# Arthur151/ROMP

Hardware: NVIDIA H100
Metric: frames/sec 512x512 ROMP-HRNet32 (whole hot path) (higher is better)
Workload: dtype bf16

## Files before the change

romp_b200/_lib.py:

```python
from __future__ import annotations

import ctypes as C
import os
import subprocess
import sys

HERE = os.path.dirname(os.path.abspath(__file__))
ROOT = os.path.dirname(HERE)
LIB_PATH = os.path.join(HERE, "lib", "libb200romp.so")
CSRC = os.path.join(HERE, "csrc")
SOURCES = ["net.cu", "conv_simt.cu", "conv_tc.cu", "conv_block_tc.cu", "conv_stem_tc.cu", "conv1d_tc.cu", "parse.cu", "smpl.cu", "smpl_blend_tc.cu", "project.cu", "bev.cu", "pack.cu", "preproc.cu", "temporal.cu", "resnet_ops.cu"]

F32, BF16, U8 = 0, 1, 2
ENGINE_AUTO, ENGINE_SIMT, ENGINE_WGMMA, ENGINE_TF32 = 0, 1, 2, 3
ENGINE_TCGEN05 = ENGINE_WGMMA


class ConvDesc(C.Structure):
    _fields_ = [(n, C.c_int) for n in (
        "in_", "in_c_off", "out", "out_c_off", "res", "res_c_off", "res_broadcast", "cin", "cout",
        "ksize", "stride", "relu", "upsample", "input_norm", "pow_channel", "engine")]


class SumDesc(C.Structure):
    _fields_ = [("out", C.c_int), ("base", C.c_int), ("n_terms", C.c_int), ("term", C.c_int * 4), ("up", C.c_int * 4),
                ("relu", C.c_int), ("term_c_off", C.c_int * 4)]


class BevWeights(C.Structure):
    _fields_ = [(n, C.POINTER(C.c_float)) for n in (
        "center_ref", "cam_ref", "coordmap", "anchors", "embed", "w0", "b0", "w1", "b1", "w2", "b2")]


NVCC_FLAGS = ["-Xcompiler", "-fPIC", "-std=c++17", "-O3", "-lineinfo", "-gencode", "arch=compute_90a,code=sm_90a"]
OBJ_DIR = os.path.join(HERE, "lib", "obj")


def _nvcc():
    return os.environ.get("NVCC", "/usr/local/cuda/bin/nvcc")


def nvcc_command(out_path=LIB_PATH):
    return [_nvcc(), "-shared"] + NVCC_FLAGS + ["-o", out_path] + [os.path.join(CSRC, s) for s in SOURCES]

# ... 143 lines not shown
```

romp_b200/csrc/conv_tc.cu:

```cuda
#include <mutex>

#include "conv_tc.cuh"
#include "tc_device.cuh"

namespace b200romp {

thread_local int g_tc_pdl_override = -1;

constexpr int kTcThreads = 384;
constexpr int kMaxRings = 2;

__host__ __device__ constexpr int s2_row_bytes(int cin, int eb) { return cin * eb >= 512 ? 64 : (cin * eb < 128 ? cin * eb : 128); }

__host__ __device__ constexpr int tc_num_rings(int stages) { return stages >= 4 ? kMaxRings : 1; }
__host__ __device__ constexpr int tc_ring_size(int stages, int ring) { return tc_num_rings(stages) == 1 ? stages : (stages + 1 - ring) / 2; }
__host__ __device__ constexpr int tc_ring_base(int stages, int ring) { return ring ? (stages + 1) / 2 : 0; }

template <int MODE, int CIN, int NT, int EB>
struct TcCfg {
  static constexpr bool S2 = MODE == 2;
  static constexpr int KS = MODE == 1 ? 1 : 3;
  static constexpr int TAPS = KS * KS;
  static constexpr int PAD = KS / 2;
  static constexpr int ROWB = S2 ? s2_row_bytes(CIN, EB) : tc_row_bytes(KS, CIN, EB);
// ... 263 lines not shown
  return true;
}

bool tc_conv_supported(const ConvParams& p, int ksize, int stride) {
  TcConvPlan plan;
  return tc_shape_supported(p, ksize, stride) && tc_tile(p, ksize, stride, &plan);
}

template <int MODE, int CIN, int NT, int EB>
static int launch_inst(const TcConvPlan& plan, const ConvParams& p, cudaStream_t stream, bool set_attr_only) {
  if (set_attr_only) {
    B2R_CUDA_OK(cudaFuncSetAttribute(conv_tc_kernel<MODE, CIN, NT, EB, true>, cudaFuncAttributeMaxDynamicSharedMemorySize, 227 * 1024));
    B2R_CUDA_OK(cudaFuncSetAttribute(conv_tc_kernel<MODE, CIN, NT, EB, false>, cudaFuncAttributeMaxDynamicSharedMemorySize, 227 * 1024));
    return B200ROMP_OK;
  }
  auto kern = p.cout % NT == 0 && tc_nhwc_out(p, p.cout) ? conv_tc_kernel<MODE, CIN, NT, EB, false> : conv_tc_kernel<MODE, CIN, NT, EB, true>;
  CUtensorMap tm;
  memcpy(&tm, plan.tmap_in, sizeof(tm));
  S2Maps s2;
  memcpy(&s2, plan.tmap_s2, sizeof(s2));
  const int tiles_x = p.Wout / 8, tiles_y = p.Hout / 16;
  const int num_tiles = tiles_x * tiles_y * p.B;
  dim3 grid(std::min(plan.grid_x, num_tiles), plan.grid_y);
  B2R_CUDA_OK(tc_launch(kern, grid, kTcThreads, plan.smem_bytes, stream, tm, s2, p, reinterpret_cast<const uint8_t*>(plan.d_wpack), tiles_x,
                        tiles_y, num_tiles, plan.stages, plan.kmask));
  return B200ROMP_OK;
}

static int dispatch(const TcConvPlan& plan, const ConvParams& p, cudaStream_t stream, bool attr) {
  const int mode = plan.kind == 32 ? 2 : plan.kind / 10;
#define B2R_CASE(M, C, N, E) \
  if (mode == M && plan.cin == C && plan.nt == N && plan.eb == E) return launch_inst<M, C, N, E>(plan, p, stream, attr);
  B2R_CASE(3, 32, 32, 2) B2R_CASE(3, 32, 64, 2) B2R_CASE(3, 64, 32, 2) B2R_CASE(3, 64, 64, 2) B2R_CASE(3, 128, 32, 2) B2R_CASE(3, 128, 64, 2)
  B2R_CASE(3, 256, 32, 2) B2R_CASE(3, 256, 64, 2)
  B2R_CASE(1, 32, 32, 2) B2R_CASE(1, 32, 64, 2) B2R_CASE(1, 64, 32, 2) B2R_CASE(1, 64, 64, 2) B2R_CASE(1, 128, 32, 2) B2R_CASE(1, 128, 64, 2)
  B2R_CASE(1, 256, 32, 2) B2R_CASE(1, 256, 64, 2)
  B2R_CASE(2, 32, 32, 2) B2R_CASE(2, 32, 64, 2) B2R_CASE(2, 64, 32, 2) B2R_CASE(2, 64, 64, 2) B2R_CASE(2, 128, 32, 2) B2R_CASE(2, 256, 32, 2)
  B2R_CASE(3, 32, 32, 4) B2R_CASE(3, 32, 64, 4) B2R_CASE(3, 64, 32, 4) B2R_CASE(3, 64, 64, 4) B2R_CASE(3, 128, 32, 4) B2R_CASE(3, 256, 16, 4)
  B2R_CASE(1, 32, 32, 4) B2R_CASE(1, 32, 64, 4) B2R_CASE(1, 64, 32, 4) B2R_CASE(1, 64, 64, 4) B2R_CASE(1, 128, 32, 4) B2R_CASE(1, 128, 64, 4)
  B2R_CASE(1, 256, 32, 4) B2R_CASE(1, 256, 64, 4)
  B2R_CASE(2, 32, 32, 4) B2R_CASE(2, 32, 64, 4) B2R_CASE(2, 64, 32, 4) B2R_CASE(2, 128, 32, 4)
#undef B2R_CASE
  set_error("conv_tc: no instantiation for mode %d cin%d nt%d eb%d", mode, plan.cin, plan.nt, plan.eb);
  return B200ROMP_EINVAL;
}

int tc_conv_prepare(const ConvParams& p, int ksize, int stride, const float* w_oihw, int sm_count, TcConvPlan* plan,
                    std::vector<void*>* allocs) {
  PFN_encodeTiled encode = tc_get_encode();
  if (!encode) {
    set_error("conv_tc: cuTensorMapEncodeTiled is unavailable");
    return B200ROMP_ECUDA;
  }
  if (!tc_tile(p, ksize, stride, plan)) {
    set_error("conv_tc: k%d s%d cin%d does not fit shared memory", ksize, stride, p.cin);
    return B200ROMP_EINVAL;
  }
  const int eb = plan->eb, rowb = tc_rowb(ksize, stride, p.cin, eb), cw = rowb / eb;
  plan->grid_y = (p.cout + plan->nt - 1) / plan->nt;
  plan->grid_x = std::max(1, sm_count / plan->grid_y);
  int rc = tc_pack_weights(w_oihw, p.cin, p.cout, ksize * ksize, plan->nt, &plan->d_wpack, allocs, rowb, eb);
  if (rc) return rc;
  const CUtensorMapDataType dtype = eb == 2 ? CU_TENSOR_MAP_DATA_TYPE_BFLOAT16 : CU_TENSOR_MAP_DATA_TYPE_FLOAT32;
  const CUtensorMapSwizzle swizzle = rowb == 128 ? CU_TENSOR_MAP_SWIZZLE_128B : CU_TENSOR_MAP_SWIZZLE_64B;
  if (stride == 2) {
    const cuuint64_t C = (cuuint64_t)p.in_C;
    const cuuint64_t gdim[5] = {2 * C, (cuuint64_t)p.Win / 2, 2, (cuuint64_t)p.Hin / 2, (cuuint64_t)p.B};
    const cuuint64_t E = (cuuint64_t)eb;
    const cuuint64_t gstr[4] = {2 * C * E, (cuuint64_t)p.Win * C * E, 2 * (cuuint64_t)p.Win * C * E, (cuuint64_t)p.Hin * p.Win * C * E};
    const cuuint32_t estr[5] = {1, 1, 1, 1, 1};
    for (int i = 0; i < 4; ++i) {
      const cuuint32_t box[5] = {(cuuint32_t)cw, (cuuint32_t)((i & 1) ? 8 : 9), 1, (cuuint32_t)(i < 2 ? 17 : 16), 1};
      CUtensorMap tm;
      CUresult cr = encode(&tm, dtype, 5, const_cast<void*>(p.in), gdim, gstr, box, estr, CU_TENSOR_MAP_INTERLEAVE_NONE, swizzle,
                           CU_TENSOR_MAP_L2_PROMOTION_L2_128B, CU_TENSOR_MAP_FLOAT_OOB_FILL_NONE);
      if (cr != CUDA_SUCCESS) {
        set_error("conv_tc: cuTensorMapEncodeTiled (stride 2) failed with %d", (int)cr);
        return B200ROMP_ECUDA;
      }
      memcpy(plan->tmap_s2[i], &tm, sizeof(tm));
    }
  } else {
    const int hh = 16 + 2 * (ksize / 2), hw = 8 + 2 * (ksize / 2);
    CUtensorMap tm;
    const cuuint64_t gdim[4] = {(cuuint64_t)p.cin, (cuuint64_t)p.Win, (cuuint64_t)p.Hin, (cuuint64_t)p.B};
    const cuuint64_t gstr[3] = {(cuuint64_t)p.in_C * eb, (cuuint64_t)p.Win * p.in_C * eb, (cuuint64_t)p.Hin * p.Win * p.in_C * eb};
    const cuuint32_t box[4] = {(cuuint32_t)cw, (cuuint32_t)hw, (cuuint32_t)hh, 1};
    const cuuint32_t estr[4] = {1, 1, 1, 1};
    void* base = const_cast<uint8_t*>(static_cast<const uint8_t*>(p.in) + (size_t)p.in_c_off * eb);
    CUresult cr = encode(&tm, dtype, 4, base, gdim, gstr, box, estr, CU_TENSOR_MAP_INTERLEAVE_NONE, swizzle,
                         CU_TENSOR_MAP_L2_PROMOTION_L2_128B, CU_TENSOR_MAP_FLOAT_OOB_FILL_NONE);
    if (cr != CUDA_SUCCESS) {
      set_error("conv_tc: cuTensorMapEncodeTiled failed with %d", (int)cr);
      return B200ROMP_ECUDA;
    }
    memcpy(plan->tmap_in, &tm, sizeof(tm));
  }
  return dispatch(*plan, p, nullptr, true);
}

int tc_conv_launch(const TcConvPlan& plan, const ConvParams& p, cudaStream_t stream) { return dispatch(plan, p, stream, false); }

}
```

romp_b200/csrc/conv_tc.cuh:

```cuda
#pragma once
#include <cuda.h>

#include <string>
#include <vector>

#include "common.cuh"

namespace b200romp {

struct S2Maps {
  CUtensorMap m[4];
};

struct TcConvPlan {
  int kind = 0;
  int cin = 0, cout = 0, nt = 0;
  int eb = 2;
  int grid_x = 0, grid_y = 0, stages = 0;
  int smem_bytes = 0;
  void* d_wpack = nullptr;
  alignas(64) unsigned char tmap_in[128];
  alignas(64) unsigned char tmap_s2[4][128];
  unsigned kmask = 0xFFFFFFFFu;
  const void* encoded_in = nullptr;
  int encoded_batch = 0;
  void* d_wpack2 = nullptr;
  const float* d_bias1 = nullptr;
  int fold = 0;
  std::string describe() const;
};

bool tc_conv_supported(const ConvParams& p, int ksize, int stride);
int tc_conv_prepare(const ConvParams& p, int ksize, int stride, const float* w_oihw, int sm_count, TcConvPlan* plan,
                    std::vector<void*>* allocs);
int tc_conv_launch(const TcConvPlan& plan, const ConvParams& p, cudaStream_t stream);
bool tc_conv1d_supported(const ConvParams& p);
int tc_conv1d_prepare(const ConvParams& p, const float* w_oi3, int sm_count, TcConvPlan* plan, std::vector<void*>* allocs);
int tc_conv1d_launch(TcConvPlan& plan, const ConvParams& p, cudaStream_t stream);
bool tc_stem_supported(const ConvParams& p, int ksize, int stride);
int tc_stem_prepare(const ConvParams& p, const float* w_oihw, int sm_count, TcConvPlan* plan, std::vector<void*>* allocs);
int tc_stem_launch(const TcConvPlan& plan, const ConvParams& p, cudaStream_t stream);
bool tc_block_supported(const ConvParams& p);
int tc_block_prepare(const ConvParams& p, const float* w1_oihw, const float* b1, const float* w2_oihw, int sm_count,
                     TcConvPlan* plan, std::vector<void*>* allocs);
int tc_block_launch(const TcConvPlan& plan, const ConvParams& p, cudaStream_t stream);

}
```

romp_b200/csrc/net.cu:

```cuda
#include <stdarg.h>
#include <stdlib.h>
#include <string.h>

#include <algorithm>
#include <map>
#include <mutex>
#include <vector>

#include "common.cuh"
#include "conv_tc.cuh"

namespace b200romp {

static thread_local std::string g_last_error;

void set_error(const char* fmt, ...) {
  char buf[1024];
  va_list ap;
  va_start(ap, fmt);
  vsnprintf(buf, sizeof(buf), fmt, ap);
  va_end(ap);
  g_last_error = buf;
}

struct Tensor {
  int H, W, C, dtype, nchw, external;
  void* ptr = nullptr;
  bool constant = false;
  int first_def = -1, last_use = -1;
  size_t frame_bytes() const { return (size_t)H * W * C * dtype_size(dtype); }
};

enum class Kernel { Sum, MaxPool, Simt, Generic7x7, Deconv4x4, Wgmma, WgmmaStem, WgmmaConv1d, WgmmaBlock };

struct Op {
  Kernel kernel = Kernel::Simt;
  b200romp_sum_desc sum;
  b200romp_conv_desc d;
  std::vector<float> w_host, b_host;
  float* d_w_simt = nullptr;
  float* d_bias = nullptr;
  int coutPad = 0;
  TcConvPlan tc;
  int lane = 0;
  int mid = -1;
  std::vector<float> w2_host, b2_host;
};

static bool on_wgmma(Kernel k) { return k == Kernel::Wgmma || k == Kernel::WgmmaStem || k == Kernel::WgmmaConv1d || k == Kernel::WgmmaBlock; }

}

using namespace b200romp;

struct b200romp_net {
  int device = 0;
  int sm_count = 132;
  bool finalized = false;
  int max_batch = 0;
  std::vector<Tensor> tensors;
  std::vector<Op> ops;
  std::vector<void*> device_allocs;
  char* workspace = nullptr;
  size_t workspace_bytes = 0;
  struct GraphKey {
    int batch;
    std::vector<void*> ext;
    bool operator<(const GraphKey& o) const { return batch != o.batch ? batch < o.batch : ext < o.ext; }
  };
  std::map<GraphKey, cudaGraphExec_t> graphs;
  bool use_graph = true;
  static constexpr int kLanes = 4;
  cudaStream_t lane_stream[kLanes] = {nullptr, nullptr, nullptr, nullptr};
  std::vector<cudaEvent_t> op_done;
  cudaEvent_t fork_ev = nullptr;
  bool use_lanes = false;
};

static int fill_params(const b200romp_net* net, const Op& op, int batch, bool allow_unbound, ConvParams* out) {
  const b200romp_conv_desc& d = op.d;
  const Tensor& ti = net->tensors[d.in];
  const Tensor& to = net->tensors[d.out];
// ... 190 lines not shown
  for (int k = 0; k < p.n_terms; ++k) {
    const Tensor& tt = net->tensors[op.sum.term[k]];
    B2R_REQUIRE(tt.ptr, "sum op: unbound term tensor");
    p.term[k] = tt.ptr; p.term_dt[k] = tt.dtype; p.up[k] = op.sum.up[k];
    p.term_C[k] = tt.C; p.term_c_off[k] = op.sum.term_c_off[k];
  }
  p.B = batch; p.H = to.H; p.W = to.W; p.C = to.C; p.relu = op.sum.relu;
  *out = p;
  return B200ROMP_OK;
}

static int enqueue_op(b200romp_net* net, Op& op, int batch, cudaStream_t stream) {
  ConvParams p;
  if (op.kernel != Kernel::Sum && op.kernel != Kernel::MaxPool) {
    int rc = fill_params(net, op, batch, false, &p);
    if (rc) return rc;
  }
  switch (op.kernel) {
    case Kernel::Sum: {
      SumParams sp;
      int rc = fill_sum_params(net, op, batch, &sp);
      return rc ? rc : launch_fuse_sum(sp, stream);
    }
    case Kernel::MaxPool: {
      const Tensor& ti = net->tensors[op.d.in];
      const Tensor& to = net->tensors[op.d.out];
      B2R_REQUIRE(ti.ptr && to.ptr, "maxpool op: unbound tensor");
      return launch_maxpool3x3s2(ti.ptr, to.ptr, ti.dtype, batch, ti.H, ti.W, ti.C, stream);
    }
    case Kernel::Simt: return launch_conv_simt(p, op.d.ksize, op.d.stride, stream);
    case Kernel::Generic7x7: return launch_conv_generic(p, 7, op.d.stride, stream);
    case Kernel::Deconv4x4: return launch_deconv4x4s2(p, stream);
    case Kernel::Wgmma: return tc_conv_launch(op.tc, p, stream);
    case Kernel::WgmmaStem: return tc_stem_launch(op.tc, p, stream);
    case Kernel::WgmmaConv1d: return tc_conv1d_launch(op.tc, p, stream);
    case Kernel::WgmmaBlock: return tc_block_launch(op.tc, p, stream);
  }
  return B200ROMP_EINVAL;
}

static int upload(b200romp_net* net, const std::vector<float>& v, float** d) {
  B2R_CUDA_OK(cudaMalloc(d, v.size() * sizeof(float)));
  net->device_allocs.push_back(*d);
  B2R_CUDA_OK(cudaMemcpy(*d, v.data(), v.size() * sizeof(float), cudaMemcpyHostToDevice));
  return B200ROMP_OK;
}

static bool fold_eligible(const b200romp_net* net, const Op& op) {
  static const bool off = [] { const char* e = getenv("B200ROMP_TC_NO_FOLD"); return e && e[0] == '1'; }();
  const b200romp_conv_desc& d = op.d;
  const Tensor& ti = net->tensors[d.in];
  const Tensor& to = net->tensors[d.out];
  if (off || d.ksize != 3 || d.stride != 1 || d.upsample != 1 || d.cin != 32 || d.cout != 32) return false;
  if (ti.C != 32 || to.C != 32 || d.in_c_off || d.out_c_off || ti.external || to.external) return false;
  if (ti.dtype != B200ROMP_BF16 || to.dtype != B200ROMP_BF16 || to.nchw || d.pow_channel >= 0 || d.input_norm) return false;
  if (ti.W % 16 != 0 || ti.H % 16 != 0) return false;
  if (d.res >= 0) {
    const Tensor& tr = net->tensors[d.res];
    if (tr.C != 32 || d.res_c_off || d.res_broadcast || tr.dtype != B200ROMP_BF16 || tr.external) return false;
  }
  return true;
}

static void fold_pixel_pairs(std::vector<float>* w, std::vector<float>* b) {
  std::vector<float> w2((size_t)64 * 64 * 9, 0.f), b2(64);
  for (int dx = 0; dx < 2; ++dx)
// ... 73 lines not shown
          f.w2_host = std::move(b.w_host);
          f.b2_host = std::move(b.b_host);
          fused.push_back(std::move(f));
          ++i;
          continue;
        }
      }
    }
    fused.push_back(std::move(a));
  }
  net->ops = std::move(fused);
}

static int choose_kernel(const b200romp_net* net, int i, Op& op) {
  const b200romp_conv_desc& d = op.d;
  const Tensor& ti = net->tensors[d.in];
  const Tensor& to = net->tensors[d.out];
  if (d.ksize == 7 || d.ksize == 42) {
    op.kernel = d.ksize == 7 ? Kernel::Generic7x7 : Kernel::Deconv4x4;
    return B200ROMP_OK;
  }
  op.kernel = Kernel::Simt;
  const bool forced = d.engine == B200ROMP_ENGINE_WGMMA;
  const bool stem = ti.dtype == B200ROMP_U8 && d.cin == 3 && d.ksize == 3 && d.stride == 2;
  if (!forced && !(d.engine == B200ROMP_ENGINE_TF32 && ti.dtype == B200ROMP_F32) &&
      !(d.engine == B200ROMP_ENGINE_AUTO && (ti.dtype == B200ROMP_BF16 || stem)))
    return B200ROMP_OK;
  ConvParams p;
  fill_params(net, op, net->max_batch, true, &p);
  if (stem) {
    if (!to.external && d.res < 0 && tc_stem_supported(p, d.ksize, d.stride)) op.kernel = Kernel::WgmmaStem;
  } else if (d.ksize == 13) {
    if (tc_conv1d_supported(p)) op.kernel = Kernel::WgmmaConv1d;
  } else if (!ti.external && tc_conv_supported(p, d.ksize, d.stride)) {
    op.kernel = Kernel::Wgmma;
    op.tc.fold = fold_eligible(net, op);
  }
  if (forced && op.kernel == Kernel::Simt) {
    set_error("op %d: tensor-core engine forced but shape unsupported", i);
    return B200ROMP_EINVAL;
  }
  return B200ROMP_OK;
}

static int prepare_op(b200romp_net* net, Op& op) {
  if (op.kernel == Kernel::Sum || op.kernel == Kernel::MaxPool) return B200ROMP_OK;
  const b200romp_conv_desc& d = op.d;
  std::vector<float> w = std::move(op.w_host), b = std::move(op.b_host), w2 = std::move(op.w2_host), b2 = std::move(op.b2_host);
  if (op.tc.fold) {
    fold_pixel_pairs(&w, &b);
    if (op.kernel == Kernel::WgmmaBlock) fold_pixel_pairs(&w2, &b2);
  }
  std::vector<float> bias = op.kernel == Kernel::WgmmaBlock ? b2 : b;
  op.coutPad = ((int)bias.size() + 63) / 64 * 64;
  bias.resize(op.coutPad, 0.f);
  int rc = upload(net, bias, &op.d_bias);
  if (rc) return rc;
  ConvParams p;
  fill_params(net, op, net->max_batch, true, &p);
  switch (op.kernel) {
    case Kernel::Simt:
    case Kernel::Generic7x7:
    case Kernel::Deconv4x4: {
      const int taps = conv_taps(d.ksize);
      std::vector<float> packed((size_t)taps * d.cin * op.coutPad, 0.f);
      for (int co = 0; co < d.cout; ++co)
        for (int ci = 0; ci < d.cin; ++ci)
          for (int t = 0; t < taps; ++t)
            packed[((size_t)t * d.cin + ci) * op.coutPad + co] =
                d.ksize == 42 ? w[((size_t)ci * d.cout + co) * taps + t] : w[((size_t)co * d.cin + ci) * taps + t];
      return upload(net, packed, &op.d_w_simt);
    }
    case Kernel::Wgmma:
      if (op.tc.fold) op.tc.kmask = fold_kmask();
      return tc_conv_prepare(p, d.ksize, d.stride, w.data(), net->sm_count, &op.tc, &net->device_allocs);
    case Kernel::WgmmaStem: return tc_stem_prepare(p, w.data(), net->sm_count, &op.tc, &net->device_allocs);
    case Kernel::WgmmaConv1d: return tc_conv1d_prepare(p, w.data(), net->sm_count, &op.tc, &net->device_allocs);
    case Kernel::WgmmaBlock: return tc_block_prepare(p, w.data(), b.data(), w2.data(), net->sm_count, &op.tc, &net->device_allocs);
    default: return B200ROMP_OK;
  }
}

int b200romp_net_finalize(b200romp_net* net, int max_batch) {
  B2R_REQUIRE(net && !net->finalized && max_batch > 0, "finalize: bad arguments");
  B2R_CUDA_OK(cudaSetDevice(net->device));
  fuse_basic_blocks(net);
  const int nT = (int)net->tensors.size(), nO = (int)net->ops.size();
  for (int i = 0; i < nO; ++i) {
    const b200romp_conv_desc& d = net->ops[i].d;
    Tensor& to = net->tensors[d.out];
    if (to.first_def < 0) to.first_def = i;
    to.last_use = std::max(to.last_use, i);
    net->tensors[d.in].last_use = std::max(net->tensors[d.in].last_use, i);
    if (d.res >= 0) net->tensors[d.res].last_use = std::max(net->tensors[d.res].last_use, i);
    if (net->ops[i].kernel == Kernel::Sum)
      for (int k = 0; k < net->ops[i].sum.n_terms; ++k) {
        Tensor& tt = net->tensors[net->ops[i].sum.term[k]];
        B2R_REQUIRE(tt.external || tt.constant || (tt.first_def >= 0 && tt.first_def < i), "op %d sums tensor %d before it is written", i, net->ops[i].sum.term[k]);
        tt.last_use = std::max(tt.last_use, i);
      }
  }
  for (int i = 0; i < nO; ++i) {
    const b200romp_conv_desc& d = net->ops[i].d;
    const Tensor& ti = net->tensors[d.in];
    B2R_REQUIRE(ti.external || ti.constant || (ti.first_def >= 0 && ti.first_def < i), "op %d reads tensor %d before it is written", i, d.in);
    if (d.res >= 0) {
      const Tensor& tr = net->tensors[d.res];
      B2R_REQUIRE(tr.external || tr.constant || (tr.first_def >= 0 && tr.first_def < i), "op %d adds tensor %d before it is written", i, d.res);
// ... 305 lines not shown
```

romp_b200/csrc/tc_device.cuh:

```cuda
#pragma once
#include <cuda.h>

#include <vector>

#include "conv_tc.cuh"

namespace b200romp {

__device__ __forceinline__ uint32_t smem_u32(const void* p) { return (uint32_t)__cvta_generic_to_shared(p); }

__device__ __forceinline__ void mbar_init(uint64_t* bar, uint32_t count) {
  asm volatile("mbarrier.init.shared::cta.b64 [%0], %1;" ::"r"(smem_u32(bar)), "r"(count) : "memory");
}
__device__ __forceinline__ void mbar_arrive_expect_tx(uint64_t* bar, uint32_t bytes) {
  asm volatile("mbarrier.arrive.expect_tx.shared::cta.b64 _, [%0], %1;" ::"r"(smem_u32(bar)), "r"(bytes) : "memory");
}
__device__ __forceinline__ void mbar_arrive(uint64_t* bar) {
  asm volatile("mbarrier.arrive.shared::cta.b64 _, [%0];" ::"r"(smem_u32(bar)) : "memory");
}
__device__ __forceinline__ bool mbar_try_wait(uint64_t* bar, uint32_t parity) {
  uint32_t ok;
  asm volatile(
      "{\n\t.reg .pred p;\n\t"
      "mbarrier.try_wait.parity.shared::cta.b64 p, [%1], %2;\n\t"
// ... 20 lines not shown
__device__ __forceinline__ void fence_barrier_init() { asm volatile("fence.mbarrier_init.release.cluster;" ::: "memory"); }
__device__ __forceinline__ void fence_proxy_async() { asm volatile("fence.proxy.async.shared::cta;" ::: "memory"); }
__device__ __forceinline__ void wg_bar_sync(int id) { asm volatile("bar.sync %0, 128;" ::"r"(id) : "memory"); }

__device__ __forceinline__ uint64_t l2_policy_stream() {
  uint64_t pol;
  asm volatile("createpolicy.fractional.L2::evict_normal.b64 %0, 1.0;" : "=l"(pol));
  return pol;
}
__device__ __forceinline__ void tma_load_3d(void* dst, const CUtensorMap* map, uint64_t* bar, int c0, int c1, int c2, uint64_t pol) {
  asm volatile(
      "cp.async.bulk.tensor.3d.shared::cluster.global.mbarrier::complete_tx::bytes.L2::cache_hint [%0], [%1, {%3, %4, %5}], [%2], %6;"
      ::"r"(smem_u32(dst)), "l"(map), "r"(smem_u32(bar)), "r"(c0), "r"(c1), "r"(c2), "l"(pol)
      : "memory");
}
__device__ __forceinline__ void tma_load_4d(void* dst, const CUtensorMap* map, uint64_t* bar, int c0, int c1, int c2, int c3, uint64_t pol) {
  asm volatile(
      "cp.async.bulk.tensor.4d.shared::cluster.global.mbarrier::complete_tx::bytes.L2::cache_hint [%0], [%1, {%3, %4, %5, %6}], [%2], %7;"
      ::"r"(smem_u32(dst)), "l"(map), "r"(smem_u32(bar)), "r"(c0), "r"(c1), "r"(c2), "r"(c3), "l"(pol)
      : "memory");
}
__device__ __forceinline__ void tma_load_5d(void* dst, const CUtensorMap* map, uint64_t* bar, int c0, int c1, int c2, int c3,
                                            int c4, uint64_t pol) {
  asm volatile(
      "cp.async.bulk.tensor.5d.shared::cluster.global.mbarrier::complete_tx::bytes.L2::cache_hint [%0], [%1, {%3, %4, %5, %6, %7}], [%2], %8;"
      ::"r"(smem_u32(dst)), "l"(map), "r"(smem_u32(bar)), "r"(c0), "r"(c1), "r"(c2), "r"(c3), "r"(c4), "l"(pol)
      : "memory");
}
__device__ __forceinline__ void bulk_copy_g2s(void* dst, const void* src, uint32_t bytes, uint64_t* bar) {
  asm volatile("cp.async.bulk.shared::cluster.global.mbarrier::complete_tx::bytes [%0], [%1], %2, [%3];"
               ::"r"(smem_u32(dst)), "l"(src), "r"(bytes), "r"(smem_u32(bar))
               : "memory");
}

__device__ __forceinline__ void wgmma_fence() { asm volatile("wgmma.fence.sync.aligned;" ::: "memory"); }
__device__ __forceinline__ void wgmma_commit() { asm volatile("wgmma.commit_group.sync.aligned;" ::: "memory"); }
template <int N>
__device__ __forceinline__ void wgmma_wait() { asm volatile("wgmma.wait_group.sync.aligned %0;" ::"n"(N) : "memory"); }

#define B2R_WG_R8(i) "+f"(d[i + 0]), "+f"(d[i + 1]), "+f"(d[i + 2]), "+f"(d[i + 3]), "+f"(d[i + 4]), "+f"(d[i + 5]), "+f"(d[i + 6]), "+f"(d[i + 7])
__device__ __forceinline__ void wgmma_n16(float (&d)[8], uint64_t a, uint64_t b, uint32_t scale_d, bool tf32) {
  if (!tf32)
    asm volatile(
        "{\n\t.reg .pred p;\n\tsetp.ne.b32 p, %10, 0;\n\t"
        "wgmma.mma_async.sync.aligned.m64n16k16.f32.bf16.bf16 {%0, %1, %2, %3, %4, %5, %6, %7}, %8, %9, p, 1, 1, 0, 0;\n\t}"
        : B2R_WG_R8(0)
        : "l"(a), "l"(b), "r"(scale_d)
        : "memory");
  else
    asm volatile(
        "{\n\t.reg .pred p;\n\tsetp.ne.b32 p, %10, 0;\n\t"
        "wgmma.mma_async.sync.aligned.m64n16k8.f32.tf32.tf32 {%0, %1, %2, %3, %4, %5, %6, %7}, %8, %9, p, 1, 1;\n\t}"
        : B2R_WG_R8(0)
        : "l"(a), "l"(b), "r"(scale_d)
        : "memory");
}
__device__ __forceinline__ void wgmma_n32(float (&d)[16], uint64_t a, uint64_t b, uint32_t scale_d, bool tf32) {
  if (!tf32)
    asm volatile(
        "{\n\t.reg .pred p;\n\tsetp.ne.b32 p, %18, 0;\n\t"
        "wgmma.mma_async.sync.aligned.m64n32k16.f32.bf16.bf16 {%0, %1, %2, %3, %4, %5, %6, %7, %8, %9, %10, %11, %12, %13, %14, %15}, "
        "%16, %17, p, 1, 1, 0, 0;\n\t}"
        : B2R_WG_R8(0), B2R_WG_R8(8)
        : "l"(a), "l"(b), "r"(scale_d)
        : "memory");
  else
    asm volatile(
        "{\n\t.reg .pred p;\n\tsetp.ne.b32 p, %18, 0;\n\t"
        "wgmma.mma_async.sync.aligned.m64n32k8.f32.tf32.tf32 {%0, %1, %2, %3, %4, %5, %6, %7, %8, %9, %10, %11, %12, %13, %14, %15}, "
        "%16, %17, p, 1, 1;\n\t}"
        : B2R_WG_R8(0), B2R_WG_R8(8)
        : "l"(a), "l"(b), "r"(scale_d)
        : "memory");
}
__device__ __forceinline__ void wgmma_n64(float (&d)[32], uint64_t a, uint64_t b, uint32_t scale_d, bool tf32) {
  if (!tf32)
    asm volatile(
        "{\n\t.reg .pred p;\n\tsetp.ne.b32 p, %34, 0;\n\t"
        "wgmma.mma_async.sync.aligned.m64n64k16.f32.bf16.bf16 {%0, %1, %2, %3, %4, %5, %6, %7, %8, %9, %10, %11, %12, %13, %14, "
        "%15, %16, %17, %18, %19, %20, %21, %22, %23, %24, %25, %26, %27, %28, %29, %30, %31}, %32, %33, p, 1, 1, 0, 0;\n\t}"
        : B2R_WG_R8(0), B2R_WG_R8(8), B2R_WG_R8(16), B2R_WG_R8(24)
        : "l"(a), "l"(b), "r"(scale_d)
        : "memory");
  else
    asm volatile(
        "{\n\t.reg .pred p;\n\tsetp.ne.b32 p, %34, 0;\n\t"
        "wgmma.mma_async.sync.aligned.m64n64k8.f32.tf32.tf32 {%0, %1, %2, %3, %4, %5, %6, %7, %8, %9, %10, %11, %12, %13, %14, "
        "%15, %16, %17, %18, %19, %20, %21, %22, %23, %24, %25, %26, %27, %28, %29, %30, %31}, %32, %33, p, 1, 1;\n\t}"
        : B2R_WG_R8(0), B2R_WG_R8(8), B2R_WG_R8(16), B2R_WG_R8(24)
        : "l"(a), "l"(b), "r"(scale_d)
        : "memory");
}
#undef B2R_WG_R8
template <int NT, int EB>
__device__ __forceinline__ void wgmma_any(float (&d)[NT / 2], uint64_t a, uint64_t b, uint32_t scale_d) {
  if constexpr (NT == 64) wgmma_n64(d, a, b, scale_d, EB == 4);
  else if constexpr (NT == 32) wgmma_n32(d, a, b, scale_d, EB == 4);
  else wgmma_n16(d, a, b, scale_d, EB == 4);
}

constexpr uint32_t kSw128 = 1, kSw64 = 2;
__device__ __forceinline__ uint64_t make_smem_desc(uint32_t addr, uint32_t sbo_bytes, uint32_t layout) {
  return (uint64_t)((addr & 0x3FFFF) >> 4) | ((uint64_t)1 << 16) | ((uint64_t)(sbo_bytes >> 4) << 32) | ((uint64_t)layout << 62);
}
__host__ __device__ constexpr uint32_t tc_layout(int row_bytes) { return row_bytes == 128 ? kSw128 : kSw64; }

__host__ __device__ constexpr int tc_row_bytes(int ksize, int cin, int eb) {
  return (ksize == 3 && cin >= 128) ? 64 : (cin * eb < 128 ? cin * eb : 128);
}

__device__ __forceinline__ uint32_t tf32_rna(uint32_t x) {
  uint32_t y;
  asm("cvt.rna.tf32.f32 %0, %1;" : "=r"(y) : "r"(x));
  return y;
}
__device__ __forceinline__ void tf32_round_smem(uint8_t* base, int bytes, int t, int nthreads) {
  const uint32_t s0 = smem_u32(base);
  for (int off = t * 16; off < bytes; off += nthreads * 16) {
    uint32_t a, b, c, d;
    asm volatile("ld.shared.v4.b32 {%0, %1, %2, %3}, [%4];" : "=r"(a), "=r"(b), "=r"(c), "=r"(d) : "r"(s0 + off));
    a = tf32_rna(a); b = tf32_rna(b); c = tf32_rna(c); d = tf32_rna(d);
    asm volatile("st.shared.v4.b32 [%4], {%0, %1, %2, %3};" ::"r"(a), "r"(b), "r"(c), "r"(d), "r"(s0 + off) : "memory");
  }
}
// ... 115 lines not shown
        const float b0 = __ldg(bias + c), b1 = __ldg(bias + c + 1);
#pragma unroll
        for (int e = 0; e < 2; ++e) {
          const int m = 64 * h + 16 * w + (l >> 2) + 8 * e;
          wg_store2(p, n, linear ? y0 : y0 + (m >> 3), linear ? x0 + m : x0 + (m & 7), c, acc[h][4 * j + 2 * e] + b0,
                    acc[h][4 * j + 2 * e + 1] + b1);
        }
      }
    }
  }
}

template <typename... KArgs, typename... Args>
static inline cudaError_t tc_launch(void (*kern)(KArgs...), dim3 grid, int threads, int smem_bytes, cudaStream_t stream, Args&&... args) {
  static const bool pdl_default = [] { const char* e = getenv("B200ROMP_NO_PDL"); return !(e && e[0] == '1'); }();
  const bool pdl = pdl_default && g_tc_pdl_override != 0;
  cudaLaunchConfig_t cfg = {};
  cfg.gridDim = grid;
  cfg.blockDim = dim3(threads);
  cfg.dynamicSmemBytes = (size_t)smem_bytes;
  cfg.stream = stream;
  cudaLaunchAttribute at[1];
  at[0].id = cudaLaunchAttributeProgrammaticStreamSerialization;
  at[0].val.programmaticStreamSerializationAllowed = 1;
  cfg.attrs = at;
  cfg.numAttrs = pdl ? 1 : 0;
  return cudaLaunchKernelEx(&cfg, kern, static_cast<KArgs>(args)...);
}

typedef CUresult (*PFN_encodeTiled)(CUtensorMap*, CUtensorMapDataType, cuuint32_t, void*, const cuuint64_t*, const cuuint64_t*,
                                    const cuuint32_t*, const cuuint32_t*, CUtensorMapInterleave, CUtensorMapSwizzle,
                                    CUtensorMapL2promotion, CUtensorMapFloatOOBfill);
PFN_encodeTiled tc_get_encode();
int tc_pack_weights(const float* w_oihw, int cin, int cout, int taps, int nt, void** d_out, std::vector<void*>* allocs, int rowb, int eb);
float tc_round_tf32_host(float w);

}
```

Baseline: 2687.

## Add warp-specialized N=128 WGMMA kernel for deep 3x3 convs sharing weight stages

Adds a dedicated 3x3 stride-1 bf16 conv kernel for cin 128/256 with cout a multiple of 128. It uses two consumer warpgroups, each working on its own 16x8 output tile, which share a deep ring of streamed weight stages, plus per-consumer halo TMA producers and setmaxnreg register rebalancing. The wider n128 tile and shared weight fetch are meant to cut weight traffic and raise tensor-core utilisation on the low-resolution HRNet branches. The risks are lower occupancy from a single large-smem block per SM, the lag handshake between consumers stalling them, and removal of the old cin256/nt64 instantiation.

Measured after the change: 2727, median of 6. +1.5%, better.

```diff
diff --git a/romp_b200/_lib.py b/romp_b200/_lib.py
--- a/romp_b200/_lib.py
+++ b/romp_b200/_lib.py
@@ -9,7 +9,7 @@
 ROOT = os.path.dirname(HERE)
 LIB_PATH = os.path.join(HERE, "lib", "libb200romp.so")
 CSRC = os.path.join(HERE, "csrc")
-SOURCES = ["net.cu", "conv_simt.cu", "conv_tc.cu", "conv_block_tc.cu", "conv_stem_tc.cu", "conv1d_tc.cu", "parse.cu", "smpl.cu", "smpl_blend_tc.cu", "project.cu", "bev.cu", "pack.cu", "preproc.cu", "temporal.cu", "resnet_ops.cu"]
+SOURCES = ["net.cu", "conv_simt.cu", "conv_tc.cu", "conv_deep_tc.cu", "conv_block_tc.cu", "conv_stem_tc.cu", "conv1d_tc.cu", "parse.cu", "smpl.cu", "smpl_blend_tc.cu", "project.cu", "bev.cu", "pack.cu", "preproc.cu", "temporal.cu", "resnet_ops.cu"]
 
 F32, BF16, U8 = 0, 1, 2
 ENGINE_AUTO, ENGINE_SIMT, ENGINE_WGMMA, ENGINE_TF32 = 0, 1, 2, 3
diff --git a/romp_b200/csrc/conv_deep_tc.cu b/romp_b200/csrc/conv_deep_tc.cu
--- /dev/null
+++ b/romp_b200/csrc/conv_deep_tc.cu
@@ -0,0 +1,207 @@
+#include "conv_tc.cuh"
+#include "tc_device.cuh"
+
+namespace b200romp {
+
+namespace {
+constexpr int kThreads = 384;
+constexpr int kNT = 128;
+constexpr int kRowB = 64;
+constexpr int kCW = kRowB / 2;
+constexpr int kHaloPayload = 18 * 10 * kRowB;
+constexpr int kHaloBytes = 12 * 1024;
+constexpr int kWBytes = kNT * kRowB;
+constexpr int kConsumers = 2;
+constexpr int kHaloStages = 2;
+constexpr int kBarBytes = 1024;
+constexpr int kWStages = (227 * 1024 - 1024 - kBarBytes - kConsumers * kHaloStages * kHaloBytes) / kWBytes;
+constexpr int kLag = 18;
+constexpr int kSmemBytes = 1024  + kConsumers * kHaloStages * kHaloBytes + kWStages * kWBytes + kBarBytes;
+static_assert(kSmemBytes <= 227 * 1024, "deep conv stages exceed shared memory");
+static_assert((2 * kConsumers * kHaloStages + 2 * kWStages + 1) * 8 <= kBarBytes, "barriers exceed their block");
+static_assert(kLag < kWStages, "the lag must leave consumer 0 a free weight stage");
+}
+
+template <int CIN>
+__global__ void __launch_bounds__(kThreads, 1)
+conv_deep_tc_kernel(const __grid_constant__ CUtensorMap tmap, const ConvParams p, const uint8_t* __restrict__ wpack, int tiles_x,
+                    int tiles_y, int num_tiles) {
+  constexpr int KCH = CIN / kCW;
+  static_assert(kLag < 9 * KCH, "consumer 0 must reach the lag inside its first tile");
+  extern __shared__ uint8_t smem_raw[];
+  uint8_t* smem = reinterpret_cast<uint8_t*>((reinterpret_cast<uintptr_t>(smem_raw) + 1023) & ~(uintptr_t)1023);
+  uint8_t* sH = smem;
+  uint8_t* sW = sH + kConsumers * kHaloStages * kHaloBytes;
+  uint64_t* hfull = reinterpret_cast<uint64_t*>(sW + kWStages * kWBytes);
+  uint64_t* hempty = hfull + kConsumers * kHaloStages;
+  uint64_t* wfull = hempty + kConsumers * kHaloStages;
+  uint64_t* wempty = wfull + kWStages;
+  uint64_t* go = wempty + kWStages;
+
+  const int warp = threadIdx.x >> 5;
+  if (threadIdx.x == 0) {
+    for (int i = 0; i < kConsumers * kHaloStages; ++i) {
+      mbar_init(&hfull[i], 1);
+      mbar_init(&hempty[i], 4);
+    }
+    for (int i = 0; i < kWStages; ++i) {
+      mbar_init(&wfull[i], 1);
+      mbar_init(&wempty[i], 4 * kConsumers);
+    }
+    mbar_init(go, 4);
+    fence_barrier_init();
+  }
+  __syncthreads();
+  pdl_trigger();
+  const int per_frame = tiles_x * tiles_y;
+  const int n_pairs = (num_tiles + 1) / 2;
+
+  if (warp < 4) {
+    setmaxnreg_dec<40>();
+    if (warp < kConsumers) {
+      const int g = warp;
+      const bool leader = (threadIdx.x & 31) == 0;
+      pdl_wait();
+      const uint64_t pol = l2_policy_stream();
+      int hs = 0;
+      uint32_t hph = 0;
+      for (int pair = blockIdx.x; pair < n_pairs; pair += gridDim.x) {
+        const int tile = min(2 * pair + g, num_tiles - 1);
+        const int n = tile / per_frame, rem = tile % per_frame;
+        for (int c = 0; c < KCH; ++c) {
+          const int hidx = g * kHaloStages + hs;
+          mbar_wait(&hempty[hidx], hph ^ 1);
+          if (leader) {
+            mbar_arrive_expect_tx(&hfull[hidx], kHaloPayload);
+            tma_load_4d(sH + (size_t)hidx * kHaloBytes, &tmap, &hfull[hidx], c * kCW, (rem % tiles_x) * 8 - 1, (rem / tiles_x) * 16 - 1,
+                        n, pol);
+          }
+          __syncwarp();
+          if (++hs == kHaloStages) { hs = 0; hph ^= 1; }
+        }
+      }
+    } else if (warp == kConsumers) {
+      const bool leader = (threadIdx.x & 31) == 0;
+      const uint8_t* wsrc = wpack + (size_t)blockIdx.y * 9 * KCH * kWBytes;
+      int ws = 0;
+      uint32_t wph = 0;
+      for (int pair = blockIdx.x; pair < n_pairs; pair += gridDim.x) {
+        for (int c = 0; c < KCH; ++c) {
+          for (int tap = 0; tap < 9; ++tap) {
+            mbar_wait(&wempty[ws], wph ^ 1);
+            if (leader) {
+              mbar_arrive_expect_tx(&wfull[ws], kWBytes);
+              bulk_copy_g2s(sW + (size_t)ws * kWBytes, wsrc + (size_t)(tap * KCH + c) * kWBytes, kWBytes, &wfull[ws]);
+            }
+            __syncwarp();
+            if (++ws == kWStages) { ws = 0; wph ^= 1; }
+          }
+        }
+      }
+    }
+  } else {
+    setmaxnreg_inc<232>();
+    const int g = (warp >> 2) - 1, t = threadIdx.x & 127, wlane = threadIdx.x & 31;
+    pdl_wait();
+    if (g == 1) mbar_wait(go, 0);
+    const uint32_t h_base = smem_u32(sH + (size_t)g * kHaloStages * kHaloBytes), w_base = smem_u32(sW);
+    int hs = 0, ws = 0, done = 0;
+    uint32_t hph = 0, wph = 0;
+    for (int pair = blockIdx.x; pair < n_pairs; pair += gridDim.x) {
+      const int tile = 2 * pair + g;
+      const int tc = min(tile, num_tiles - 1);
+      const int n = tc / per_frame, rem = tc % per_frame;
+      const int y0 = (rem / tiles_x) * 16, x0 = (rem % tiles_x) * 8;
+      float acc[2][kNT / 2];
+#pragma unroll
+      for (int h = 0; h < 2; ++h)
+#pragma unroll
+        for (int j = 0; j < kNT / 2; ++j) acc[h][j] = 0.f;
+      uint32_t scale_d = 0;
+      int prev_w = -1, prev_h = -1;
+      for (int c = 0; c < KCH; ++c) {
+        const int hidx = g * kHaloStages + hs;
+        mbar_wait(&hfull[hidx], hph);
+        const uint32_t a_base = h_base + (uint32_t)(hs * kHaloBytes);
+#pragma unroll
+        for (int tap = 0; tap < 9; ++tap) {
+          mbar_wait(&wfull[ws], wph);
+          const uint32_t a_tap = a_base + (uint32_t)(((tap / 3) * 10 + tap % 3) * kRowB), sbo = 10 * kRowB;
+          const uint32_t b_tap = w_base + (uint32_t)(ws * kWBytes);
+          wgmma_fence();
+#pragma unroll
+          for (int k = 0; k < kRowB / 32; ++k) {
+            const uint64_t bdesc = make_smem_desc(b_tap + k * 32, 8 * kRowB, kSw64);
+            wgmma_n128(acc[0], make_smem_desc(a_tap + k * 32, sbo, kSw64), bdesc, scale_d);
+            wgmma_n128(acc[1], make_smem_desc(a_tap + 8 * sbo + k * 32, sbo, kSw64), bdesc, scale_d);
+            scale_d = 1;
+          }
+          wgmma_commit();
+          if (prev_w >= 0) {
+            wgmma_wait<1>();
+            if (wlane == 0) {
+              mbar_arrive(&wempty[prev_w]);
+              if (prev_h >= 0) mbar_arrive(&hempty[prev_h]);
+            }
+          }
+          prev_w = ws;
+          prev_h = tap == 8 ? hidx : -1;
+          if (++ws == kWStages) { ws = 0; wph ^= 1; }
+          if (g == 0 && ++done == kLag && wlane == 0) mbar_arrive(go);
+        }
+        if (++hs == kHaloStages) { hs = 0; hph ^= 1; }
+      }
+      wgmma_wait<0>();
+      if (wlane == 0) {
+        mbar_arrive(&wempty[prev_w]);
+        mbar_arrive(&hempty[prev_h]);
+      }
+      if (tile < num_tiles) wg_epilogue<kNT, kEpiNhwc>(p, acc, p.bias, n, y0, x0, blockIdx.y * kNT, t);
+    }
+  }
+}
+
+bool tc_deep_supported(const ConvParams& p, int ksize, int stride, int sm_count) {
+  if (ksize != 3 || stride != 1 || p.in_dtype != B200ROMP_BF16 || p.input_norm) return false;
+  if (p.Hout % 16 != 0 || p.Wout % 8 != 0) return false;
+  const long long pairs = ((long long)(p.Hout / 16) * (p.Wout / 8) * p.B + 1) / 2;
+  if (4 * pairs * (p.cout / kNT) < 3LL * sm_count) return false;
+  if (p.cin != 128 && p.cin != 256) return false;
+  if (p.cout % kNT != 0 || !tc_nhwc_out(p, p.cout)) return false;
+  if (p.out_dtype != B200ROMP_BF16 && p.out_dtype != B200ROMP_F32) return false;
+  if (p.Hout != p.Hin || p.Wout != p.Win || p.Hout % 16 != 0 || p.Wout % 8 != 0) return false;
+  if (p.in_C % 8 != 0 || p.in_c_off % 8 != 0) return false;
+  if (p.out_C % 8 != 0 || p.out_c_off % 8 != 0) return false;
+  if (p.res != nullptr && (p.res_C % 8 != 0 || p.res_c_off % 8 != 0)) return false;
+  if ((reinterpret_cast<uintptr_t>(p.in) & 15) != 0) return false;
+  return true;
+}
+
+static decltype(&conv_deep_tc_kernel<256>) deep_kernel(int cin) { return cin == 128 ? conv_deep_tc_kernel<128> : conv_deep_tc_kernel<256>; }
+
+int tc_deep_prepare(const ConvParams& p, const float* w_oihw, int sm_count, TcConvPlan* plan, std::vector<void*>* allocs) {
+  plan->kind = 34;
+  plan->eb = 2;
+  plan->cin = p.cin; plan->cout = p.cout; plan->nt = kNT;
+  plan->stages = kWStages;
+  plan->smem_bytes = kSmemBytes;
+  plan->grid_y = p.cout / kNT;
+  plan->grid_x = std::max(1, sm_count / plan->grid_y);
+  B2R_CUDA_OK(cudaFuncSetAttribute(deep_kernel(p.cin), cudaFuncAttributeMaxDynamicSharedMemorySize, kSmemBytes));
+  int rc = tc_pack_weights(w_oihw, p.cin, p.cout, 9, kNT, &plan->d_wpack, allocs, kRowB, 2);
+  if (rc) return rc;
+  return tc_encode_halo_map(p, 3, kRowB, 2, plan->tmap_in);
+}
+
+int tc_deep_launch(const TcConvPlan& plan, const ConvParams& p, cudaStream_t stream) {
+  CUtensorMap tm;
+  memcpy(&tm, plan.tmap_in, sizeof(tm));
+  const int tiles_x = p.Wout / 8, tiles_y = p.Hout / 16;
+  const int num_tiles = tiles_x * tiles_y * p.B;
+  const int grid_x = std::min(plan.grid_x, (num_tiles + 1) / 2);
+  B2R_CUDA_OK(tc_launch(deep_kernel(plan.cin), dim3(grid_x, plan.grid_y), kThreads, plan.smem_bytes, stream, tm, p,
+                        reinterpret_cast<const uint8_t*>(plan.d_wpack), tiles_x, tiles_y, num_tiles));
+  return B200ROMP_OK;
+}
+
+}
diff --git a/romp_b200/csrc/conv_tc.cu b/romp_b200/csrc/conv_tc.cu
--- a/romp_b200/csrc/conv_tc.cu
+++ b/romp_b200/csrc/conv_tc.cu
@@ -319,7 +319,7 @@
 #define B2R_CASE(M, C, N, E) \
   if (mode == M && plan.cin == C && plan.nt == N && plan.eb == E) return launch_inst<M, C, N, E>(plan, p, stream, attr);
   B2R_CASE(3, 32, 32, 2) B2R_CASE(3, 32, 64, 2) B2R_CASE(3, 64, 32, 2) B2R_CASE(3, 64, 64, 2) B2R_CASE(3, 128, 32, 2) B2R_CASE(3, 128, 64, 2)
-  B2R_CASE(3, 256, 32, 2) B2R_CASE(3, 256, 64, 2)
+  B2R_CASE(3, 256, 32, 2)
   B2R_CASE(1, 32, 32, 2) B2R_CASE(1, 32, 64, 2) B2R_CASE(1, 64, 32, 2) B2R_CASE(1, 64, 64, 2) B2R_CASE(1, 128, 32, 2) B2R_CASE(1, 128, 64, 2)
   B2R_CASE(1, 256, 32, 2) B2R_CASE(1, 256, 64, 2)
   B2R_CASE(2, 32, 32, 2) B2R_CASE(2, 32, 64, 2) B2R_CASE(2, 64, 32, 2) B2R_CASE(2, 64, 64, 2) B2R_CASE(2, 128, 32, 2) B2R_CASE(2, 256, 32, 2)
@@ -368,24 +368,37 @@
       memcpy(plan->tmap_s2[i], &tm, sizeof(tm));
     }
   } else {
-    const int hh = 16 + 2 * (ksize / 2), hw = 8 + 2 * (ksize / 2);
-    CUtensorMap tm;
-    const cuuint64_t gdim[4] = {(cuuint64_t)p.cin, (cuuint64_t)p.Win, (cuuint64_t)p.Hin, (cuuint64_t)p.B};
-    const cuuint64_t gstr[3] = {(cuuint64_t)p.in_C * eb, (cuuint64_t)p.Win * p.in_C * eb, (cuuint64_t)p.Hin * p.Win * p.in_C * eb};
-    const cuuint32_t box[4] = {(cuuint32_t)cw, (cuuint32_t)hw, (cuuint32_t)hh, 1};
-    const cuuint32_t estr[4] = {1, 1, 1, 1};
-    void* base = const_cast<uint8_t*>(static_cast<const uint8_t*>(p.in) + (size_t)p.in_c_off * eb);
-    CUresult cr = encode(&tm, dtype, 4, base, gdim, gstr, box, estr, CU_TENSOR_MAP_INTERLEAVE_NONE, swizzle,
-                         CU_TENSOR_MAP_L2_PROMOTION_L2_128B, CU_TENSOR_MAP_FLOAT_OOB_FILL_NONE);
-    if (cr != CUDA_SUCCESS) {
-      set_error("conv_tc: cuTensorMapEncodeTiled failed with %d", (int)cr);
-      return B200ROMP_ECUDA;
-    }
-    memcpy(plan->tmap_in, &tm, sizeof(tm));
+    rc = tc_encode_halo_map(p, ksize, rowb, eb, plan->tmap_in);
+    if (rc) return rc;
   }
   return dispatch(*plan, p, nullptr, true);
 }
 
+int tc_encode_halo_map(const ConvParams& p, int ksize, int rowb, int eb, void* tmap_out) {
+  PFN_encodeTiled encode = tc_get_encode();
+  if (!encode) {
+    set_error("conv_tc: cuTensorMapEncodeTiled is unavailable");
+    return B200ROMP_ECUDA;
+  }
+  const int hh = 16 + 2 * (ksize / 2), hw = 8 + 2 * (ksize / 2), cw = rowb / eb;
+  const CUtensorMapDataType dtype = eb == 2 ? CU_TENSOR_MAP_DATA_TYPE_BFLOAT16 : CU_TENSOR_MAP_DATA_TYPE_FLOAT32;
+  const CUtensorMapSwizzle swizzle = rowb == 128 ? CU_TENSOR_MAP_SWIZZLE_128B : CU_TENSOR_MAP_SWIZZLE_64B;
+  CUtensorMap tm;
+  const cuuint64_t gdim[4] = {(cuuint64_t)p.cin, (cuuint64_t)p.Win, (cuuint64_t)p.Hin, (cuuint64_t)p.B};
+  const cuuint64_t gstr[3] = {(cuuint64_t)p.in_C * eb, (cuuint64_t)p.Win * p.in_C * eb, (cuuint64_t)p.Hin * p.Win * p.in_C * eb};
+  const cuuint32_t box[4] = {(cuuint32_t)cw, (cuuint32_t)hw, (cuuint32_t)hh, 1};
+  const cuuint32_t estr[4] = {1, 1, 1, 1};
+  void* base = const_cast<uint8_t*>(static_cast<const uint8_t*>(p.in) + (size_t)p.in_c_off * eb);
+  CUresult cr = encode(&tm, dtype, 4, base, gdim, gstr, box, estr, CU_TENSOR_MAP_INTERLEAVE_NONE, swizzle,
+                       CU_TENSOR_MAP_L2_PROMOTION_L2_128B, CU_TENSOR_MAP_FLOAT_OOB_FILL_NONE);
+  if (cr != CUDA_SUCCESS) {
+    set_error("conv_tc: cuTensorMapEncodeTiled failed with %d", (int)cr);
+    return B200ROMP_ECUDA;
+  }
+  memcpy(tmap_out, &tm, sizeof(tm));
+  return B200ROMP_OK;
+}
+
 int tc_conv_launch(const TcConvPlan& plan, const ConvParams& p, cudaStream_t stream) { return dispatch(plan, p, stream, false); }
 
 }
diff --git a/romp_b200/csrc/conv_tc.cuh b/romp_b200/csrc/conv_tc.cuh
--- a/romp_b200/csrc/conv_tc.cuh
+++ b/romp_b200/csrc/conv_tc.cuh
@@ -40,6 +40,9 @@
 bool tc_stem_supported(const ConvParams& p, int ksize, int stride);
 int tc_stem_prepare(const ConvParams& p, const float* w_oihw, int sm_count, TcConvPlan* plan, std::vector<void*>* allocs);
 int tc_stem_launch(const TcConvPlan& plan, const ConvParams& p, cudaStream_t stream);
+bool tc_deep_supported(const ConvParams& p, int ksize, int stride, int sm_count);
+int tc_deep_prepare(const ConvParams& p, const float* w_oihw, int sm_count, TcConvPlan* plan, std::vector<void*>* allocs);
+int tc_deep_launch(const TcConvPlan& plan, const ConvParams& p, cudaStream_t stream);
 bool tc_block_supported(const ConvParams& p);
 int tc_block_prepare(const ConvParams& p, const float* w1_oihw, const float* b1, const float* w2_oihw, int sm_count,
                      TcConvPlan* plan, std::vector<void*>* allocs);
diff --git a/romp_b200/csrc/net.cu b/romp_b200/csrc/net.cu
--- a/romp_b200/csrc/net.cu
+++ b/romp_b200/csrc/net.cu
@@ -31,7 +31,7 @@
   size_t frame_bytes() const { return (size_t)H * W * C * dtype_size(dtype); }
 };
 
-enum class Kernel { Sum, MaxPool, Simt, Generic7x7, Deconv4x4, Wgmma, WgmmaStem, WgmmaConv1d, WgmmaBlock };
+enum class Kernel { Sum, MaxPool, Simt, Generic7x7, Deconv4x4, Wgmma, WgmmaDeep, WgmmaStem, WgmmaConv1d, WgmmaBlock };
 
 struct Op {
   Kernel kernel = Kernel::Simt;
@@ -47,7 +47,7 @@
   std::vector<float> w2_host, b2_host;
 };
 
-static bool on_wgmma(Kernel k) { return k == Kernel::Wgmma || k == Kernel::WgmmaStem || k == Kernel::WgmmaConv1d || k == Kernel::WgmmaBlock; }
+static bool on_wgmma(Kernel k) { return k == Kernel::Wgmma || k == Kernel::WgmmaDeep || k == Kernel::WgmmaStem || k == Kernel::WgmmaConv1d || k == Kernel::WgmmaBlock; }
 
 }
 
@@ -304,6 +304,7 @@
     case Kernel::Generic7x7: return launch_conv_generic(p, 7, op.d.stride, stream);
     case Kernel::Deconv4x4: return launch_deconv4x4s2(p, stream);
     case Kernel::Wgmma: return tc_conv_launch(op.tc, p, stream);
+    case Kernel::WgmmaDeep: return tc_deep_launch(op.tc, p, stream);
     case Kernel::WgmmaStem: return tc_stem_launch(op.tc, p, stream);
     case Kernel::WgmmaConv1d: return tc_conv1d_launch(op.tc, p, stream);
     case Kernel::WgmmaBlock: return tc_block_launch(op.tc, p, stream);
@@ -443,6 +444,8 @@
     if (!to.external && d.res < 0 && tc_stem_supported(p, d.ksize, d.stride)) op.kernel = Kernel::WgmmaStem;
   } else if (d.ksize == 13) {
     if (tc_conv1d_supported(p)) op.kernel = Kernel::WgmmaConv1d;
+  } else if (!ti.external && tc_deep_supported(p, d.ksize, d.stride, net->sm_count)) {
+    op.kernel = Kernel::WgmmaDeep;
   } else if (!ti.external && tc_conv_supported(p, d.ksize, d.stride)) {
     op.kernel = Kernel::Wgmma;
     op.tc.fold = fold_eligible(net, op);
@@ -485,6 +488,7 @@
     case Kernel::Wgmma:
       if (op.tc.fold) op.tc.kmask = fold_kmask();
       return tc_conv_prepare(p, d.ksize, d.stride, w.data(), net->sm_count, &op.tc, &net->device_allocs);
+    case Kernel::WgmmaDeep: return tc_deep_prepare(p, w.data(), net->sm_count, &op.tc, &net->device_allocs);
     case Kernel::WgmmaStem: return tc_stem_prepare(p, w.data(), net->sm_count, &op.tc, &net->device_allocs);
     case Kernel::WgmmaConv1d: return tc_conv1d_prepare(p, w.data(), net->sm_count, &op.tc, &net->device_allocs);
     case Kernel::WgmmaBlock: return tc_block_prepare(p, w.data(), b.data(), w2.data(), net->sm_count, &op.tc, &net->device_allocs);
diff --git a/romp_b200/csrc/tc_device.cuh b/romp_b200/csrc/tc_device.cuh
--- a/romp_b200/csrc/tc_device.cuh
+++ b/romp_b200/csrc/tc_device.cuh
@@ -76,6 +76,10 @@
                ::"r"(smem_u32(dst)), "l"(src), "r"(bytes), "r"(smem_u32(bar))
                : "memory");
 }
+template <int R>
+__device__ __forceinline__ void setmaxnreg_dec() { asm volatile("setmaxnreg.dec.sync.aligned.u32 %0;" ::"n"(R)); }
+template <int R>
+__device__ __forceinline__ void setmaxnreg_inc() { asm volatile("setmaxnreg.inc.sync.aligned.u32 %0;" ::"n"(R)); }
 
 __device__ __forceinline__ void wgmma_fence() { asm volatile("wgmma.fence.sync.aligned;" ::: "memory"); }
 __device__ __forceinline__ void wgmma_commit() { asm volatile("wgmma.commit_group.sync.aligned;" ::: "memory"); }
@@ -134,6 +138,17 @@
         : B2R_WG_R8(0), B2R_WG_R8(8), B2R_WG_R8(16), B2R_WG_R8(24)
         : "l"(a), "l"(b), "r"(scale_d)
         : "memory");
+}
+__device__ __forceinline__ void wgmma_n128(float (&d)[64], uint64_t a, uint64_t b, uint32_t scale_d) {
+  asm volatile(
+      "{\n\t.reg .pred p;\n\tsetp.ne.b32 p, %66, 0;\n\t"
+      "wgmma.mma_async.sync.aligned.m64n128k16.f32.bf16.bf16 {%0, %1, %2, %3, %4, %5, %6, %7, %8, %9, %10, %11, %12, %13, %14, "
+      "%15, %16, %17, %18, %19, %20, %21, %22, %23, %24, %25, %26, %27, %28, %29, %30, %31, %32, %33, %34, %35, %36, %37, %38, "
+      "%39, %40, %41, %42, %43, %44, %45, %46, %47, %48, %49, %50, %51, %52, %53, %54, %55, %56, %57, %58, %59, %60, %61, %62, "
+      "%63}, %64, %65, p, 1, 1, 0, 0;\n\t}"
+      : B2R_WG_R8(0), B2R_WG_R8(8), B2R_WG_R8(16), B2R_WG_R8(24), B2R_WG_R8(32), B2R_WG_R8(40), B2R_WG_R8(48), B2R_WG_R8(56)
+      : "l"(a), "l"(b), "r"(scale_d)
+      : "memory");
 }
 #undef B2R_WG_R8
 template <int NT, int EB>
@@ -315,6 +330,7 @@
                                     const cuuint32_t*, const cuuint32_t*, CUtensorMapInterleave, CUtensorMapSwizzle,
                                     CUtensorMapL2promotion, CUtensorMapFloatOOBfill);
 PFN_encodeTiled tc_get_encode();
+int tc_encode_halo_map(const ConvParams& p, int ksize, int rowb, int eb, void* tmap_out);
 int tc_pack_weights(const float* w_oihw, int cin, int cout, int taps, int nt, void** d_out, std::vector<void*>* allocs, int rowb, int eb);
 float tc_round_tf32_host(float w);
 
```
